# zenustech/zpc

Hardware: AMD Instinct MI355X
Metric: particle*steps/s (P2G+G2P) (higher is better)
Workload: dtype f32

## Files before the change

include/zs_rocm.h:

```cpp
#ifndef ZS_ROCM_H
#define ZS_ROCM_H
#include <stdbool.h>
#include <stddef.h>
#include <stdint.h>

#ifdef __cplusplus
extern "C" {
#endif

#if defined(__GNUC__)
#  define ZS_ROCM_EXPORT __attribute__((visibility("default")))
#else
#  define ZS_ROCM_EXPORT
#endif

typedef struct zs_rocm_policy zs_rocm_policy;

ZS_ROCM_EXPORT zs_rocm_policy *policy__device(void);
ZS_ROCM_EXPORT void del_policy__device(zs_rocm_policy *);
ZS_ROCM_EXPORT void zs_rocm_policy_sync(zs_rocm_policy *, int sync);
ZS_ROCM_EXPORT void zs_rocm_policy_profile(zs_rocm_policy *, int profile);
ZS_ROCM_EXPORT void zs_rocm_policy_device(zs_rocm_policy *, int procid);
ZS_ROCM_EXPORT void zs_rocm_policy_stream(zs_rocm_policy *, int streamid);
ZS_ROCM_EXPORT void zs_rocm_policy_listen(zs_rocm_policy *, int incomingProc, int incomingStreamid);
// ... 570 lines not shown
ZS_ROCM_EXPORT int zs_rocm_mesh_system_blocks(zs_rocm_policy *, const zs_rocm_mesh *, const zs_rocm_mesh_system *, float *scratch, float *elastic,
                                              float *barrier, float *friction, float *combined, float *inverse, int *status);
ZS_ROCM_EXPORT int zs_rocm_mesh_system_multiply(zs_rocm_policy *, const zs_rocm_mesh *, const zs_rocm_mesh_system *, float *scratch,
                                                const float *x, float *q);
ZS_ROCM_EXPORT int zs_rocm_mesh_system_solve(zs_rocm_policy *, const zs_rocm_mesh *, const zs_rocm_mesh_system *, float *scratch,
                                             const float *inverse, const float *b, float *x, int maxIters, float tol, float relTol,
                                             int checkEvery, void *record);
ZS_ROCM_EXPORT int zs_rocm_mesh_potential_sizes(const zs_rocm_mesh *, const zs_rocm_mesh_system *, size_t *sizes);
ZS_ROCM_EXPORT int zs_rocm_mesh_potential_evaluate(zs_rocm_policy *, const zs_rocm_mesh *, const zs_rocm_mesh_system *, const float *target,
                                                   const float *start, const float *verts, float *scratch, float *energies, double *parts,
                                                   float *grad, int *status);
ZS_ROCM_EXPORT int zs_rocm_mesh_potential_line_search(zs_rocm_policy *, const zs_rocm_mesh *, const zs_rocm_mesh_system *, const float *target,
                                                      const float *start, const float *verts, const float *dir, float tMax,
                                                      const float *tMaxDev, float c1, float shrink, int maxTrials, int checkEvery,
                                                      float *scratch, float *energies, float *x, void *record);
ZS_ROCM_EXPORT int zs_rocm_mesh_ccd(zs_rocm_policy *, const zs_rocm_mesh *, const float *verts, const float *dir, const int *ptPairs, size_t npt,
                                    const int *eePairs, size_t nee, float slack, float tMax, int maxIter, float *ptToi, float *eeToi,
                                    float *tMin, int *status);
#define ZS_ROCM_SLOT_STATUS_WORDS (8 + 2 * 256)
ZS_ROCM_EXPORT size_t zs_rocm_mpm_slot_outbox_bytes(size_t nbins, int outboxCap, int which);
ZS_ROCM_EXPORT void zs_rocm_mpm_build_neighbors27(zs_rocm_policy *, const zs_rocm_bht_3 *, int *nbr27 , int keyStride);
ZS_ROCM_EXPORT int zs_rocm_mpm_slot_particles(zs_rocm_policy *, const zs_rocm_bht_3 *, zs_rocm_attr pos, size_t n, float dx, int side,
                                              int keyIsOrigin, int K, const float *src, float *dst, int C, unsigned *cellMask, int *status);
ZS_ROCM_EXPORT size_t zs_rocm_mpm_slot_list(zs_rocm_policy *, const unsigned *cellMask, size_t nbins, int K, int *slots);
typedef struct zs_rocm_slot_storage {
  unsigned *cellMask;
  int K;
  const int *nbr;
  const int *nbr27;
  int *moverCount;
  unsigned *claim;
  float *moverRec;
  int outboxCap;
  int *status;
  const unsigned char *blockEdge;
} zs_rocm_slot_storage;
ZS_ROCM_EXPORT void zs_rocm_mpm_partition_edge(zs_rocm_policy *, const zs_rocm_bht_3 *, unsigned char *edge , int keyStride,
                                               int lo, int hi);
ZS_ROCM_EXPORT void zs_rocm_mpm_slot_compute_sparsity(zs_rocm_policy *, const zs_rocm_bht_3 *oldTab, const unsigned *cellMask, size_t nblocksOld,
                                                      int side, int keyIsOrigin, zs_rocm_bht_3 *newTab);
ZS_ROCM_EXPORT int zs_rocm_mpm_reslot(zs_rocm_policy *, const zs_rocm_bht_3 *oldTab, const zs_rocm_bht_3 *newTab, int side, int K, int C,
                                      const float *oldBuf, float *newBuf, const unsigned *oldMask, unsigned *newMask, const float *oldGrid,
                                      float *newGrid, int *status);
ZS_ROCM_EXPORT int zs_rocm_mpm_g2p2g_slots(zs_rocm_policy *, const zs_rocm_mpm_params *, zs_rocm_particles, const zs_rocm_bht_3 *,
                                           const float *gridA, float *gridB, size_t nblocks, const zs_rocm_slot_storage *st, int writeAll,
                                           size_t blockBegin, size_t blockEnd, int finish);
// ... 62 lines not shown
                                                                    const size_t *peerOffset, const size_t *peerCount, const int *blocks,
                                                                    size_t total);
typedef struct zs_rocm_mpm_step {
  const zs_rocm_mpm_params *params;
  zs_rocm_particles particles;
  const zs_rocm_bht_3 *table;
  const float *gridA;
  float *gridB;
  size_t nblocks;
  const zs_rocm_slot_storage *storage;
  int writeAll;
  float extf[3];
  float *maxVelSqr;
  const zs_rocm_collider *collider;
  size_t nBoundary;
  zs_rocm_dist *dist;
  zs_rocm_halo_plan *plan;
  zs_rocm_policy *commPolicy;
  float *haloGrid;
  void *evTransferBegin, *evTransferEnd;
  void **evBreakdown;
  int haloChannels;
  int rangeSchedule;
  float *handoverSnapshot;
  float *gridClear;
  int gridBIsClear;
  const zs_rocm_levelset *levelset;
} zs_rocm_mpm_step;
#define ZS_ROCM_STEP_EVENTS 8
#define ZS_ROCM_RANGES_IN_TURN 0
#define ZS_ROCM_RANGES_SIDE_BY_SIDE 1
#define ZS_ROCM_RANGES_ONE_LAUNCH 2
ZS_ROCM_EXPORT int zs_rocm_mpm_step_slotted(zs_rocm_policy *, const zs_rocm_mpm_step *);

#ifdef __cplusplus
}
#endif
#endif
```

zpc_amd/_lib.py:

```python
import ctypes as C
import os

_HERE = os.path.dirname(os.path.abspath(__file__))
LIB_PATH = os.path.join(_HERE, "lib", "libzsrocm.so")
if os.environ.get("ZS_ROCM_LIB"):
    LIB_PATH = os.environ["ZS_ROCM_LIB"]
    print("[zpc_amd] using HIP library %s" % LIB_PATH, flush=True)


class Port(C.Structure):
    _fields_ = [("base", C.c_void_p), ("idx", C.c_uint32), ("numTileBits", C.c_uint32),
                ("tileMask", C.c_uint32), ("numChns", C.c_uint32)]


class HashTableView(C.Structure):
    _fields_ = [("keys", C.c_void_p), ("indices", C.c_void_p), ("status", C.c_void_p), ("activeKeys", C.c_void_p),
                ("cnt", C.c_void_p), ("tableSize", C.c_int)]


class LBvhView(C.Structure):
    _fields_ = [("orderedBvs", C.c_void_p), ("parents", C.c_void_p), ("levels", C.c_void_p), ("leafInds", C.c_void_p),
                ("auxIndices", C.c_void_p), ("numNodes", C.c_int), ("numLeaves", C.c_int)]


# ... 14 lines not shown
class BhtViewLite(C.Structure):
    _fields_ = [("keys", C.c_void_p), ("indices", C.c_void_p), ("status", C.c_void_p), ("activeKeys", C.c_void_p),
                ("cnt", C.c_void_p), ("success", C.c_void_p), ("tableSize", C.c_uint32), ("numBuckets", C.c_uint32),
                ("hf0x", C.c_uint32), ("hf0y", C.c_uint32), ("hf1x", C.c_uint32), ("hf1y", C.c_uint32),
                ("hf2x", C.c_uint32), ("hf2y", C.c_uint32)]


class Particles(C.Structure):
    _fields_ = [("mass", Port), ("pos", Port), ("vel", Port), ("C", Port), ("F", Port), ("logJp", Port),
                ("stress", Port), ("n", C.c_size_t)]


class SlotStorage(C.Structure):
    _fields_ = [("cellMask", C.c_void_p), ("K", C.c_int), ("nbr", C.c_void_p), ("nbr27", C.c_void_p), ("moverCount", C.c_void_p),
                ("claim", C.c_void_p), ("moverRec", C.c_void_p), ("outboxCap", C.c_int), ("status", C.c_void_p),
                ("blockEdge", C.c_void_p)]


class MpmStep(C.Structure):
    _fields_ = [("params", C.c_void_p), ("particles", Particles), ("table", C.c_void_p), ("gridA", C.c_void_p), ("gridB", C.c_void_p),
                ("nblocks", C.c_size_t), ("storage", C.c_void_p), ("writeAll", C.c_int), ("extf", C.c_float * 3),
                ("maxVelSqr", C.c_void_p), ("collider", C.c_void_p), ("nBoundary", C.c_size_t), ("dist", C.c_void_p),
                ("plan", C.c_void_p), ("commPolicy", C.c_void_p), ("haloGrid", C.c_void_p), ("evTransferBegin", C.c_void_p),
                ("evTransferEnd", C.c_void_p), ("evBreakdown", C.POINTER(C.c_void_p)), ("haloChannels", C.c_int), ("rangeSchedule", C.c_int), ("handoverSnapshot", C.c_void_p),
                ("gridClear", C.c_void_p), ("gridBIsClear", C.c_int), ("levelset", C.c_void_p)]


class MpmParams(C.Structure):
    _fields_ = [("model", C.c_int), ("dx", C.c_float), ("dt", C.c_float), ("volume", C.c_float), ("E", C.c_float),
                ("nu", C.c_float), ("cohesion", C.c_float), ("beta", C.c_float), ("yieldSurface", C.c_float),
                ("volCorrection", C.c_int), ("side", C.c_int), ("keyIsOrigin", C.c_int), ("yieldStress", C.c_float),
                ("xi", C.c_float), ("Msqr", C.c_float), ("hardeningOn", C.c_int), ("bulk", C.c_float), ("viscosity", C.c_float)]


_lib = None


def lib():
    global _lib
    if _lib is None:
        if not os.path.exists(LIB_PATH):
            raise RuntimeError(
                "libzsrocm.so not built (%s): run `python -m zpc_amd.build` -- zpc_amd has no CPU fallback" % LIB_PATH)
        try:
            import torch
        except ImportError:
            pass
# ... 280 lines not shown
    PP = C.POINTER(MpmParams)
    L.zs_rocm_mpm_compute_sparsity.argtypes = [vp, vp, Port, sz, f32, i32, i32]
    L.zs_rocm_mpm_enlarge_sparsity.argtypes = [vp, vp, C.POINTER(C.c_int), C.POINTER(C.c_int), i32]
    L.zs_rocm_mpm_bin_particles.argtypes = [vp, vp, Port, sz, f32, i32, i32, vp, vp, vp]
    L.zs_rocm_mpm_build_neighbors.argtypes = [vp, vp, vp, i32]
    L.zs_rocm_mpm_p2g.argtypes = [vp, PP, Particles, vp, vp, sz, vp, vp, vp]
    L.zs_rocm_mpm_owner_rank.argtypes = [vp, Port, sz, f32, C.POINTER(C.c_int), C.POINTER(C.c_int), C.POINTER(C.c_int), i32, vp]
    L.zs_rocm_mpm_owner_counts.argtypes = [vp, vp, sz, i32, vp]
    L.zs_rocm_mpm_owner_counts.restype = None
    L.zs_rocm_mpm_g2p2g.argtypes = [vp, PP, Particles, vp, vp, vp, sz, vp, vp, vp, i32]
    L.zs_rocm_mpm_g2p2g_range.argtypes = [vp, PP, Particles, vp, vp, vp, sz, vp, vp, vp, i32, sz, sz, vp]
    L.zs_rocm_mpm_g2p2g_slotted.argtypes = [vp, PP, Particles, vp, vp, vp, sz, vp, i32, vp, vp, vp, vp, vp, i32, i32, vp]
    L.zs_rocm_mpm_g2p2g_slotted.restype = i32
    L.zs_rocm_mpm_g2p2g_slotted_range.argtypes = [vp, PP, Particles, vp, vp, vp, sz, vp, i32, vp, vp, vp, vp, vp, i32, i32, vp, sz, sz, i32]
    L.zs_rocm_mpm_g2p2g_slotted_range.restype = i32
    L.zs_rocm_mpm_g2p2g_slots.argtypes = [vp, PP, Particles, vp, vp, vp, sz, C.POINTER(SlotStorage), i32, sz, sz, i32]
    L.zs_rocm_mpm_g2p2g_slots.restype = i32
    L.zs_rocm_mpm_partition_edge.argtypes = [vp, vp, vp, i32, i32, i32]
    L.zs_rocm_mpm_slot_compute_sparsity.argtypes = [vp, vp, vp, sz, i32, i32, vp]
    L.zs_rocm_mpm_reslot.argtypes = [vp, vp, vp, i32, i32, i32, vp, vp, vp, vp, vp, vp, vp]
    L.zs_rocm_mpm_reslot.restype = i32
    L.zs_rocm_mpm_step_slotted.argtypes = [vp, C.POINTER(MpmStep)]
    L.zs_rocm_mpm_step_slotted.restype = i32
    L.zs_rocm_dist_halo_plan_from_lists.argtypes = [vp, i32, i32, C.POINTER(C.c_int), C.POINTER(C.c_size_t), C.POINTER(C.c_size_t),
                                                    C.POINTER(C.c_int), sz]
    L.zs_rocm_dist_halo_plan_from_lists.restype = vp
    L.zs_rocm_mpm_g2p2g_reorder_range.argtypes = [vp, PP, Particles, Particles, vp, vp, vp, vp, sz, vp, vp, vp, i32, sz, sz, vp]
    L.zs_rocm_mpm_grid_update.argtypes = [vp, PP, vp, sz, C.POINTER(C.c_float), vp]
    L.zs_rocm_mpm_g2p.argtypes = [vp, PP, Particles, vp, vp, sz, vp, vp, vp]
    L.zs_rocm_mpm_p2c2g.argtypes = [vp, PP, Particles, vp, vp, vp, sz, i32]
    L.zs_rocm_mpm_p2c2g.restype = i32
    L.zs_rocm_mpm_pre_g2c2p.argtypes = [vp, Particles]
    L.zs_rocm_mpm_g2c2p.argtypes = [vp, PP, Particles, vp, vp, vp, sz]
    L.zs_rocm_mpm_g2c2p.restype = i32
    L.zs_rocm_mpm_post_g2c2p.argtypes = [vp, PP, Particles]
    L.zs_rocm_mpm_g2c2p_step.argtypes = [vp, PP, Particles, vp, vp, sz]
    L.zs_rocm_mpm_g2c2p_step.restype = i32
    L.zs_rocm_mpm_stress.argtypes = [vp, PP, vp, vp, sz, vp]
    L.zs_rocm_mpm_update_stress.argtypes = [vp, PP, Particles]
    L.zs_rocm_svd3.argtypes = [vp, vp, sz, vp, vp, vp]
    L.zs_rocm_nacc_msqr.argtypes = [f32]
    L.zs_rocm_nacc_msqr.restype = f32
    L.zs_rocm_collider_init.argtypes = [C.POINTER(Collider), i32, i32, C.POINTER(C.c_float), i32]
    L.zs_rocm_mpm_apply_boundary.argtypes = [vp, PP, vp, vp, sz, C.POINTER(Collider)]
    L.zs_rocm_collider_resolve.argtypes = [vp, C.POINTER(Collider), vp, vp, sz, vp]
    L.zs_rocm_mpm_implicit_force.argtypes = [vp, PP, Particles, vp, sz, vp, vp, vp, vp, vp, vp]
# ... 111 lines not shown
```

zpc_amd/csrc/common.hpp:

```cpp
#pragma once
#include <hip/hip_runtime.h>

#include <cstdint>
#include <cstdio>
#include <cstdlib>
#include <map>
#include <mutex>
#include <vector>

#include "../../include/zs_rocm.h"

namespace zsr {

constexpr int kWave = 64;
constexpr int kNumSpareStreams = 32;
constexpr size_t kCtlBytes = 132 << 10;
constexpr size_t kCtlDesc8 = 32 << 10, kCtlTicket = 128 << 10;
constexpr size_t kCtlScanTiles = 4096;

struct DeviceContext {
  int dev = 0;
  hipStream_t streams[kNumSpareStreams] = {};
  hipEvent_t events[kNumSpareStreams + 1] = {};
  int errorStatus = 0;
// ... 71 lines not shown
  unsigned cu_count();
};

template <class T> struct Port {
  T *base;
  uint32_t idx, bits, mask, chns;
  __host__ __device__ __forceinline__ size_t off(size_t i) const {
    size_t j = (size_t)idx + i;
    return (((j >> bits) * (size_t)chns) << bits) | (j & (size_t)mask);
  }
  __host__ __device__ __forceinline__ T &operator[](size_t i) const { return base[off(i)]; }
  __host__ __device__ __forceinline__ size_t cstride() const { return (size_t)mask + 1; }
  __host__ __device__ bool contiguous() const { return chns == 1; }
};
template <class T, class P> inline Port<T> make_port(const P &p) {
  return Port<T>{(T *)p.base, p.idx, p.numTileBits, p.tileMask, p.numChns};
}
template <class T> inline Port<T> contiguous_port(T *p) { return Port<T>{p, 0u, 0u, 0u, 1u}; }

inline unsigned ceil_div(size_t a, size_t b) { return (unsigned)((a + b - 1) / b); }

int mpm_g2p2g_slots_signal(zs_rocm_policy *pol, const zs_rocm_mpm_params *p, zs_rocm_particles ps, const zs_rocm_bht_3 *tab, const float *gridA,
                           float *gridB, size_t nblocks, const zs_rocm_slot_storage *st, int writeAll, size_t blockBegin, size_t blockEnd, int finish,
                           unsigned long long *signal, size_t signalBlocks, float *gridClear, float *zeroWord);
bool levelset_collider_ok(const zs_rocm_collider *collider, const zs_rocm_levelset *levelset);
void levelset_blocks_enqueue(hipStream_t stream, const zs_rocm_mpm_params *p, const int *activeKeys, float *grid, size_t nblocks,
                             const zs_rocm_collider *collider, const zs_rocm_levelset *levelset, float *dof);
bool levelset_ok(const zs_rocm_levelset *levelset);
bool transition_collider_ok(const zs_rocm_collider *collider, const zs_rocm_levelset_transition *transition);
bool transition_blocks_enqueue(hipStream_t stream, const zs_rocm_mpm_params *p, const int *activeKeys, float *grid, size_t nblocks,
                               const zs_rocm_collider *collider, const zs_rocm_levelset_transition *transition, float *dof);

}

namespace zsr {

__device__ __forceinline__ int lane_id() { return (int)(threadIdx.x & 63); }
__device__ __forceinline__ int wave_id() { return (int)(threadIdx.x >> 6); }

template <class T> __device__ __forceinline__ T shfl_down(T v, int d) { return __shfl_down(v, d, 64); }
template <class T> __device__ __forceinline__ T shfl_up(T v, int d) { return __shfl_up(v, d, 64); }
template <class T> __device__ __forceinline__ T shfl(T v, int l) { return __shfl(v, l, 64); }

__device__ __forceinline__ unsigned long long lanemask_lt() {
  return (1ull << (threadIdx.x & 63)) - 1ull;
}

// ... 10 lines not shown
```

zpc_amd/csrc/dist.hip:

```cpp
#include <rccl/rccl.h>

#include <algorithm>
#include <cstring>
#include <utility>
#include <vector>

#include "common.hpp"

struct zs_rocm_dist {
  ncclComm_t comm = nullptr;
  int rank = 0, world = 1, device = 0;
  bool broken = false;
};

namespace zsr {
static int nccl_check(ncclResult_t r, const char *what, const char *file, int line) {
  if (r == ncclSuccess) return 0;
  fprintf(stderr, "[zs_rocm | rccl] %s failed: %s at %s:%d\n", what, ncclGetErrorString(r), file, line);
  report_error(hipErrorUnknown, what, file, line);
  return -1;
}
#define ZSR_NCCL(expr)                                               \
  do {                                                               \
    if (::zsr::nccl_check((expr), #expr, __FILE__, __LINE__)) return -1; \
// ... 324 lines not shown
  return 0;
}

}
static __global__ void step_gate_kernel(const unsigned long long *signal, unsigned long long target) {
  const unsigned long long t0 = wall_clock64();
  while (__hip_atomic_load(signal, __ATOMIC_RELAXED, __HIP_MEMORY_SCOPE_AGENT) < target) {
    __builtin_amdgcn_s_sleep(64);
    if (wall_clock64() - t0 > 1000000000ull) __builtin_trap();
  }
}
extern "C" {

int zs_rocm_mpm_step_slotted(zs_rocm_policy *pol, const zs_rocm_mpm_step *a) {
  if (!pol || !a || !a->params || !a->table || !a->gridA || !a->gridB || !a->storage) return -1;
  if (a->levelset && !zsr::levelset_collider_ok(a->collider, a->levelset)) return -1;
  const size_t nb = a->nblocks;
  if (!nb) return 0;
  const int side = a->params->side;
  const size_t gridBytes = nb * (size_t)7 * side * side * side * sizeof(float);
  if (a->haloChannels < 0 || a->haloChannels > 7) return -1;
  if (a->rangeSchedule < ZS_ROCM_RANGES_IN_TURN || a->rangeSchedule > ZS_ROCM_RANGES_ONE_LAUNCH) return -1;
  if (a->rangeSchedule == ZS_ROCM_RANGES_ONE_LAUNCH && side != 8) return -1;
  float *const gridClear = side == 8 ? a->gridClear : nullptr;
  if (gridClear && (gridClear == a->gridA || gridClear == a->gridB || ((uintptr_t)gridClear & 15u))) return -1;
  if (!(gridClear && a->gridBIsClear)) zs_rocm_memset(pol, a->gridB, 0, gridBytes);
  float *const hgrid = a->haloGrid ? a->haloGrid : a->gridB;
  const bool exchange = a->dist && a->plan && a->plan->total;
  auto slots = [&](zs_rocm_policy *on, size_t b0, size_t b1, int finish, unsigned long long *signal, size_t signalBlocks) {
    return mpm_g2p2g_slots_signal(on, a->params, a->particles, a->table, a->gridA, a->gridB, nb, a->storage, a->writeAll, b0, b1, finish, signal,
                                  signalBlocks, gridClear, finish ? a->maxVelSqr : nullptr);
  };
  const int hch = a->haloChannels ? a->haloChannels : 7;
  const bool overlap = exchange && a->commPolicy && a->nBoundary > 0 && a->nBoundary < nb;
  int rc = 0;
  auto stamp = [&](void *ev) {
    if (!ev) return;
    Launch L(pol, "step: event");
    ZSR_CHECK(hipEventRecord((hipEvent_t)ev, L.stream));
  };
  auto bd = [&](int k, zs_rocm_policy *on) {
    if (!a->evBreakdown || !a->evBreakdown[k]) return;
    Launch L(on, "step: breakdown event");
    ZSR_CHECK(hipEventRecord((hipEvent_t)a->evBreakdown[k], L.stream));
  };
  stamp(a->evTransferBegin);
  bd(0, pol);
  if (overlap) {
    zs_rocm_halo_plan *p = a->plan;
    if (!p->evBoundary || !p->evDone) {
      DeviceGuard guard(p->device);
      if (!p->evBoundary && hipEventCreateWithFlags(&p->evBoundary, hipEventDisableTiming) != hipSuccess) p->evBoundary = nullptr;
      if (!p->evDone && hipEventCreateWithFlags(&p->evDone, hipEventDisableTiming) != hipSuccess) p->evDone = nullptr;
      if (!p->evBoundary || !p->evDone) {
// ... 110 lines not shown
```

zpc_amd/csrc/mpm_slot.hpp:

```cpp
#pragma once
#include "mpm_arena.hpp"
#include "mpm_fused_common.hpp"

namespace zsr {

constexpr int SL_REC = 48;
constexpr int SLR_DCELL = 14, SLR_FLAG = 15, SLR_V = 16, SLR_C = 19, SLR_PF = 28;

struct SlotArgs {
  const float *gridA;
  float *gridB;
  unsigned *cellMask;
  int K;
  const int *nbr;
  const int *nbr27;
  int *moverCount;
  unsigned *claim;
  float *moverRec;
  int *status;
  int binBase, nbins, nbinsAll;
  int cap;
  const unsigned char *blockEdge;
  unsigned long long *signal;
  int signalBlocks;
  float *gridClear;
};

constexpr int SL_NCTR = 256, SL_SENT = 8, SL_DELIVERED = 8 + SL_NCTR;
__device__ __forceinline__ int neighbour_bin8(const int *row27, int blk, int sub, int code) {
  if (code == 13) return blk * 8 + sub;
  const int dd[3] = {code / 9 - 1, (code / 3) % 3 - 1, code % 3 - 1};
  int sx[3] = {((sub >> 2) & 1) + dd[0], ((sub >> 1) & 1) + dd[1], (sub & 1) + dd[2]}, bo[3];
#pragma unroll
  for (int d = 0; d < 3; ++d) {
    bo[d] = sx[d] < 0 ? -1 : (sx[d] > 1 ? 1 : 0);
    sx[d] &= 1;
  }
  const int nb = row27[(bo[0] + 1) * 9 + (bo[1] + 1) * 3 + (bo[2] + 1)];
  return nb < 0 ? -1 : nb * 8 + ((sx[0] * 2 + sx[1]) * 2 + sx[2]);
}

constexpr int SL_NG = 9;
constexpr int SL_KMAX = 32;
constexpr int SL_ARRQ = 4;
constexpr int SL_XQ = 64;

__device__ __forceinline__ int nth_low_bit(unsigned w, unsigned t) {
  for (unsigned k = 0; k < t && w; ++k) w &= w - 1u;
  return w ? __ffs((int)w) - 1 : -1;
}
struct SlotShared {
  float *varena;
  float *parena;
  float *stage;
  unsigned long long *smask;
  unsigned short *tab;
  unsigned *mask0;
  unsigned *clr;
  unsigned *arrLocal;
  const int *nbrBlk;
  const int *nbrBin;
  unsigned (*arrCnt)[64];
  unsigned short (*arrQ)[64][SL_ARRQ];
  unsigned *xCnt;
  unsigned (*xq)[SL_XQ];
  int *outCount, *sent, *homed, *xOver;
};

template <int SIDE, class FM, class FV, class FC, class FP>
__device__ __forceinline__ void scatter_node_task(const MpmDev &mp, int node, int ch, const int (&nc)[3], const float (&d0)[3], FM fm, FV fv, FC fC,
                                                  FP fP, const int *nbrBlk, float *gridB, int *status) {
  constexpr int NC = SIDE * SIDE * SIDE;
// ... 451 lines not shown
```

zpc_amd/csrc/mpm_slotblk.hip:

```cpp
#include "mpm_slot.hpp"
#ifdef ZS_SLOTBLK_CHECK_ARENA
#include <cassert>
#endif

namespace zsr {

constexpr int SB_NG = 5;
constexpr int SB_MAXCH = 64;
constexpr int LIST_CS = 3;

struct SubGeom {
  int o[3], org[3];
};
__device__ __forceinline__ SubGeom sub_geom(const int (&borg)[3], int b) {
  SubGeom g;
  g.o[0] = ((b >> 2) & 1) * 4;
  g.o[1] = ((b >> 1) & 1) * 4;
  g.o[2] = (b & 1) * 4;
#pragma unroll
  for (int d = 0; d < 3; ++d) g.org[d] = borg[d] + g.o[d];
  return g;
}

struct BlkShared {
// ... 356 lines not shown
  constexpr int NC = 512;
  __shared__ float s_varena[3 * ArenaBlk::CH];
  __shared__ float s_parena[7 * ArenaBin8::CH];
  __shared__ float s_stage[SB_NG * G2P2G_QF * 64];
  __shared__ unsigned long long s_smask[SB_NG];
  __shared__ unsigned short s_tab[2][SL_KMAX * 64];
  __shared__ unsigned s_masks[8][64];
  __shared__ unsigned s_clr[2][64], s_arrLocal[8][64], s_arrCnt[3][64];
  __shared__ unsigned short s_arrQ[3][64][SL_ARRQ];
  __shared__ unsigned s_xCnt[3], s_xq[3][SL_XQ];
  __shared__ int s_nbrBlk[27], s_nbrBin[2][27], s_nbr8[8];
  __shared__ int s_cnt[2][4];
  __shared__ int s_total[8], s_gbase[8], s_binQ[8], s_oc[8];
  __shared__ unsigned char s_chBin[SB_MAXCH], s_chIdx[SB_MAXCH];
  __shared__ unsigned s_desc[SB_MAXCH + 5];
  __shared__ unsigned s_done, s_listDone, s_faces[2];
  __shared__ int s_sums[3], s_G;
  __shared__ float *s_clear;
  const BlkShared sh{s_varena, s_parena, s_stage, s_smask, s_tab, s_masks, s_clr, s_arrLocal, s_arrCnt, s_arrQ, s_xCnt, s_xq, s_nbrBlk, s_nbrBin, s_nbr8,
                     s_cnt, s_oc, s_desc, &s_done, &s_listDone, s_faces, s_sums};
  const int tid = threadIdx.x, lane = tid & 63, w = tid >> 6;
  const int blk = (int)blockIdx.x + A.binBase / 8;
  const int bin0 = blk * 8;
  const unsigned mask = A.cellMask[(size_t)(bin0 + w) * 64 + lane];
  s_masks[w][lane] = mask;
  s_arrLocal[w][lane] = 0u;
  {
    int n = __popc(mask);
#pragma unroll
    for (int sft = 32; sft >= 1; sft >>= 1) n += __shfl_xor(n, sft, 64);
    if (lane == 0) s_total[w] = n;
  }
  if (tid < 128) s_clr[tid >> 6][tid & 63] = 0u;
  if (tid < 192) s_arrCnt[tid >> 6][tid & 63] = 0u;
  if (tid < 3) {
    s_xCnt[tid] = 0u;
    s_sums[tid] = 0;
  }
  if (tid < 8) (&s_cnt[0][0])[tid] = 0;
  if (tid == 0) {
    s_done = 0u;
    s_listDone = 0u;
    s_clear = A.gridClear ? A.gridClear + (size_t)blk * 7 * NC : nullptr;
  }
  if (tid >= 64 && tid < 64 + 27) s_nbrBlk[tid - 64] = A.nbr27[(size_t)blk * 27 + (tid - 64)];
  if (tid >= 96 && tid < 104) s_nbr8[tid - 96] = A.nbr[(size_t)blk * 8 + (tid - 96)];
  int borg[3];
// ... 113 lines not shown
```

zpc_amd/csrc/mpm_slotted.hip:

```cpp
#include "mpm_slot.hpp"

namespace zsr {

void exclusive_scan_u32(Launch &L, const unsigned *in, size_t n, unsigned *out);

template <int SIDE>
static __global__ __launch_bounds__(256) void slot_assign_kernel(BhtDev t, Port<float> pos, size_t n, float dx, unsigned *cellCount, int K,
                                                                 int *srcOf, int *status, int kscale) {
  size_t i = (size_t)blockIdx.x * blockDim.x + threadIdx.x;
  if (i >= n) return;
  float p[3];
  load_attr<3>(pos, i, p);
  int key[3], loc[3];
#pragma unroll
  for (int d = 0; d < 3; ++d) {
    const int c = (int)floorf(p[d] * (1.0f / dx) - 0.5f);
    loc[d] = c & (SIDE - 1);
    key[d] = (c - loc[d]) / SIDE * kscale;
  }
  const int b = bht_query<3>(t, key);
  if (b < 0) {
    status[2] = 1;
    return;
  }
// ... 201 lines not shown
        C[d] = rc[SLR_C + d];
        PF[d] = rc[SLR_PF + d];
      }
      pstore<LW, 3>(ps.vel, o, v);
      pstore<LW, 9>(ps.C, o, C);
      {
        float S[STRESS_N];
        stress_pack(PF, S);
        pstore<LW, STRESS_N>(ps.stress, o, S);
      }
    }
  }
#pragma unroll
  for (int sft = 32; sft >= 1; sft >>= 1) nhomed += __shfl_xor(nhomed, sft, 64);
  if ((threadIdx.x & 63) == 0 && nhomed) atomicAdd(&status[SL_DELIVERED + (int)((bin >> 3) & (SL_NCTR - 1))], nhomed);
}

static __global__ __launch_bounds__(256) void slot_commit_kernel(unsigned *cellMask, unsigned *claim, size_t ncells, int K, float *zeroWord) {
  const size_t c = (size_t)blockIdx.x * blockDim.x + threadIdx.x;
  if (c == 0 && zeroWord) *zeroWord = 0.f;
  if (c >= ncells) return;
  const unsigned tk = claim[c], clr = claim[ncells + c];
  if (!tk && !clr) return;
  const unsigned m0 = cellMask[c];
  const unsigned kmask = K >= 32 ? 0xffffffffu : ((1u << K) - 1u);
  const unsigned n = (tk >> 16) + (tk & 0xffffu);
  unsigned rest = ~m0 & kmask, bits = 0u;
  for (unsigned k = 0; k < n && rest; ++k) {
    const unsigned b = rest & (0u - rest);
    bits |= b;
    rest ^= b;
  }
  cellMask[c] = (m0 & ~clr) | bits;
  claim[c] = 0u;
  claim[ncells + c] = 0u;
}

template <int SIDE>
static __global__ __launch_bounds__(256) void slot_sparsity_kernel(BhtDev oldT, const unsigned *cellMask, size_t ncells, int kscale, BhtDev newT) {
  const size_t c = (size_t)blockIdx.x * blockDim.x + threadIdx.x;
  const bool valid = c < ncells && cellMask[c] != 0u;
  int b[3] = {0, 0, 0};
  if (valid) {
    const size_t bin = c >> 6;
    const int lane = (int)(c & 63), blk = (int)(bin / bins_per_block<SIDE>()), sub = (int)(bin % bins_per_block<SIDE>());
    const int o[3] = {SIDE == 4 ? 0 : ((sub >> 2) & 1) * 4, SIDE == 4 ? 0 : ((sub >> 1) & 1) * 4, SIDE == 4 ? 0 : (sub & 1) * 4};
    const int l[3] = {lane >> 4, (lane >> 2) & 3, lane & 3};
#pragma unroll
    for (int d = 0; d < 3; ++d) b[d] = floordiv(oldT.activeKeys[3 * (size_t)blk + d] * (SIDE / kscale) + o[d] + l[d] - 1, SIDE) * kscale;
  }
  const int px = shfl_up(b[0], 1), py = shfl_up(b[1], 1), pz = shfl_up(b[2], 1);
  const bool pvalid = shfl_up((int)valid, 1) != 0;
  const bool dup = lane_id() != 0 && pvalid && px == b[0] && py == b[1] && pz == b[2];
  if (valid && !dup) bht_insert<3>(newT, b);
}
static __global__ __launch_bounds__(256) void reslot_map_kernel(BhtDev oldT, int nOld, BhtDev newT, int *map) {
// ... 74 lines not shown
  hipLaunchKernelGGL(slot_mask_kernel, dim3(ceil_div(ncells, 256)), dim3(256), 0, L.stream, cellMask, ncells, K);
  hipLaunchKernelGGL(slot_gather_kernel, dim3(ceil_div(nslots, 256)), dim3(256), 0, L.stream, src, dst, nslots, C, (const int *)srcOf);
  return 0;
}

size_t zs_rocm_mpm_slot_list(zs_rocm_policy *pol, const unsigned *cellMask, size_t nbins, int K, int *slots) {
  Launch L(pol, "slot_list");
  const size_t ncells = nbins * 64;
  if (!ncells) return 0;
  unsigned *cnt = (unsigned *)L.temp(sizeof(unsigned) * (ncells + 1)), *start = (unsigned *)L.temp(sizeof(unsigned) * (ncells + 1));
  ZSR_CHECK(hipMemsetAsync(cnt + ncells, 0, sizeof(unsigned), L.stream));
  hipLaunchKernelGGL(slot_popc_kernel, dim3(ceil_div(ncells, 256)), dim3(256), 0, L.stream, cellMask, ncells, cnt);
  exclusive_scan_u32(L, cnt, ncells + 1, start);
  unsigned total = 0;
  ZSR_CHECK(hipMemcpyAsync(&total, start + ncells, sizeof(unsigned), hipMemcpyDeviceToHost, L.stream));
  if (slots) hipLaunchKernelGGL(slot_emit_kernel, dim3(ceil_div(ncells, 256)), dim3(256), 0, L.stream, cellMask, (const unsigned *)start, ncells, K, slots);
  ZSR_CHECK(hipStreamSynchronize(L.stream));
  return (size_t)total;
}

int zs_rocm_mpm_g2p2g_slots(zs_rocm_policy *pol, const zs_rocm_mpm_params *p, zs_rocm_particles ps, const zs_rocm_bht_3 *tab,
                            const float *gridA, float *gridB, size_t nblocks, const zs_rocm_slot_storage *st, int writeAll,
                            size_t blockBegin, size_t blockEnd, int finish) {
  return zsr::mpm_g2p2g_slots_signal(pol, p, ps, tab, gridA, gridB, nblocks, st, writeAll, blockBegin, blockEnd, finish, nullptr, 0, nullptr, nullptr);
}
}
namespace zsr {
int mpm_g2p2g_slots_signal(zs_rocm_policy *pol, const zs_rocm_mpm_params *p, zs_rocm_particles ps, const zs_rocm_bht_3 *tab, const float *gridA,
                           float *gridB, size_t nblocks, const zs_rocm_slot_storage *st, int writeAll, size_t blockBegin, size_t blockEnd, int finish,
                           unsigned long long *signal, size_t signalBlocks, float *gridClear, float *zeroWord) {
  if (!st) return -1;
  if (signal && p->side != 8) return -1;
  if (p->side != 8) gridClear = nullptr;
  if (gridClear && (gridClear == gridA || gridClear == gridB || ((uintptr_t)gridClear & 15u))) return -1;
  unsigned *const cellMask = st->cellMask;
  const int K = st->K, outboxCap = st->outboxCap;
  const int *const nbr = st->nbr, *const nbr27 = st->nbr27;
  int *const moverCount = st->moverCount, *const status = st->status;
  unsigned *const claim = st->claim;
  float *const moverRec = st->moverRec;
  if (!nblocks) return 0;
  if (!cellMask || !nbr || !nbr27 || !moverCount || !claim || !moverRec || !status || K < 1 || K > 32 || outboxCap < 1 || outboxCap > (1 << 20)) return -1;
  if (p->model < ZS_MPM_FIXED_COROTATED || p->model > ZS_MPM_EQUATION_OF_STATE) return -1;
  if (uniform_lane_width(ps, model_uses_logjp(p->model), writeAll != 0) != 64 || (writeAll && (!ps.vel.base || !ps.C.base))) {
    fprintf(stderr, "[zs_rocm] g2p2g_slotted needs all particle attributes in one TileVector<f32, 64>\n");
    return -1;
  }
  if (blockEnd > nblocks) blockEnd = nblocks;
  Launch L(pol, "G2P2GTransfer(slotted)");
  MpmDev mp = make_dev(p);
  ParticlesDev pd = make_particles(ps);
  BhtDev t = tab->t.dev();
  const unsigned bpb = p->side == 4 ? 1u : 8u;
  const unsigned nbinsAll = (unsigned)(nblocks * bpb);
  const unsigned nbins = blockBegin < blockEnd ? (unsigned)((blockEnd - blockBegin) * bpb) : 0u;
  const SlotArgs A{gridA, gridB, cellMask, K, nbr, nbr27, moverCount, claim, moverRec, status, (int)(blockBegin * bpb), (int)nbins, (int)nbinsAll, outboxCap,
                   st->blockEdge, signal, (int)signalBlocks, gridClear};
#define CALL_REHOME3(M, WA)                                                                                                              \
  hipLaunchKernelGGL((slot_rehome_kernel<model_is_fluid(M), model_uses_logjp(M), WA>), dim3(ceil_div((size_t)nbinsAll, 32)), dim3(256), 0,  \
                     L.stream, pd, (const unsigned *)cellMask, claim, (const int *)moverCount, (const float *)moverRec, outboxCap,        \
                     (size_t)nbinsAll, K, status)
#define CALL_REHOME(SS, M)                      \
  do {                                          \
    if (writeAll) { CALL_REHOME3(M, true); }    \
    else { CALL_REHOME3(M, false); }            \
  } while (0)
  if (p->side == 8) {
    if (nbins) launch_g2p2g_slotblk(L.stream, p->model, writeAll != 0, mp, pd, t, A);
  } else if (nbins) {
#define CALL_SLOT4(SS, M)                                                                                                  \
  do {                                                                                                                     \
    if (writeAll) hipLaunchKernelGGL((g2p2g_slot_kernel<4, M, true>), dim3(nbins), dim3(512), 0, L.stream, mp, pd, t, A);  \
    else hipLaunchKernelGGL((g2p2g_slot_kernel<4, M, false>), dim3(nbins), dim3(512), 0, L.stream, mp, pd, t, A);          \
  } while (0)
    ZSR_DISPATCH_PURE_(4, p->model, CALL_SLOT4)
  }
  if (finish) ZSR_DISPATCH_PURE_(0, p->model, CALL_REHOME)
  if (finish) {
    const size_t ncells = (size_t)nbinsAll * 64;
    hipLaunchKernelGGL(slot_commit_kernel, dim3(ceil_div(ncells, 256)), dim3(256), 0, L.stream, cellMask, claim, ncells, K, zeroWord);
  }
  return 0;
}
}
extern "C" {

int zs_rocm_mpm_g2p2g_slotted_range(zs_rocm_policy *pol, const zs_rocm_mpm_params *p, zs_rocm_particles ps, const zs_rocm_bht_3 *tab,
                                    const float *gridA, float *gridB, size_t nblocks, unsigned *cellMask, int K, const int *nbr, const int *nbr27,
                                    int *moverCount, unsigned *claim, float *moverRec, int outboxCap, int writeAll, int *status,
                                    size_t blockBegin, size_t blockEnd, int finish) {
  const zs_rocm_slot_storage st{cellMask, K, nbr, nbr27, moverCount, claim, moverRec, outboxCap, status, nullptr};
  return zs_rocm_mpm_g2p2g_slots(pol, p, ps, tab, gridA, gridB, nblocks, &st, writeAll, blockBegin, blockEnd, finish);
}

int zs_rocm_mpm_g2p2g_slotted(zs_rocm_policy *pol, const zs_rocm_mpm_params *p, zs_rocm_particles ps, const zs_rocm_bht_3 *tab, const float *gridA,
                              float *gridB, size_t nblocks, unsigned *cellMask, int K, const int *nbr, const int *nbr27, int *moverCount,
                              unsigned *claim, float *moverRec, int outboxCap, int writeAll, int *status) {
  return zs_rocm_mpm_g2p2g_slotted_range(pol, p, ps, tab, gridA, gridB, nblocks, cellMask, K, nbr, nbr27, moverCount, claim, moverRec, outboxCap,
                                         writeAll, status, 0, nblocks, 1);
}

void zs_rocm_mpm_partition_edge(zs_rocm_policy *pol, const zs_rocm_bht_3 *tab, unsigned char *edge, int keyStride, int lo, int hi) {
  Launch L(pol, "partition_edge");
// ... 39 lines not shown
```

zpc_amd/mpm.py:

```python
import ctypes as C

import torch

from ._lib import lib, Port, Particles, MpmParams, SlotStorage, MpmStep
from .containers import Bht

FIXED_COROTATED, DRUCKER_PRAGER, VONMISES_FIXED_COROTATED, NACC = 0, 1, 2, 3
EQUATION_OF_STATE = 4
HAS_LOGJP = (DRUCKER_PRAGER, NACC)


class MpmTransfer:
    def __init__(self, pol, n, dx, dt, model=FIXED_COROTATED, side=4, lane_width=64, E=5e4, nu=0.4, volume=1.0,
                 cohesion=0.0, beta=1.0, yield_surface=0.816496580927726 * 2.0 * 0.5 / (3.0 - 0.5), vol_correction=True,
                 device="cuda", key_is_origin=False, aos=False, cache_stress=False, yield_stress=240e6, xi=0.8, friction_angle=45.0,
                 hardening=True, bulk=4e4, viscosity=0.0):
        self.pol, self.n, self.L, self.side = pol, int(n), int(lane_width), int(side)
        self.device = torch.device(device)
        self.model = model
        self.fluid = model == EQUATION_OF_STATE
        self.nF = 1 if self.fluid else 9
        self.nchn = 16 + self.nF + (1 if model in HAS_LOGJP else 0)
        self.off = {"m": 0, "x": 1, "v": 4, "C": 7, "F": 16, "logJp": 25}
        self.cache_stress = bool(cache_stress)
# ... 9 lines not shown
        self.buf = torch.zeros(self.tiles * self.L * self.nchn, dtype=torch.float32, device=self.device)
        self.buf2 = None
        self.drift_flag = None
        self.drift_tripped = False
        self.outside_tripped = False
        self.key_is_origin = bool(key_is_origin)
        self.kstride = side if key_is_origin else 1
        self.params = MpmParams(model, dx, dt, volume, E, nu, cohesion, beta, yield_surface, int(vol_correction), side,
                                int(self.key_is_origin), yield_stress, xi, lib().zs_rocm_nacc_msqr(friction_angle), int(hardening),
                                bulk, viscosity)
        self.table = None
        self.grid = None
        self.grid2 = self.grid3 = None
        self._clean_grid = None
        self.rotate_grids = True
        self.nblocks = 0
        self.order = self.bin_start = self.cell_count = self.nbr = None
        self.binned = False
        self.slotted = False
        self.n_slots = 0
        self.K = 0
        self.slot_record = {"sent": 0, "homed": 0, "flags": [0] * 5, "periods": 0, "edge_periods": 0, "log": []}

    def _grids_written(self):
        self._clean_grid = None

    def _zero(self, t):
        lib().zs_rocm_memset(self.pol.handle, t.data_ptr(), 0, t.numel() * t.element_size())

    def _port(self, name, buf=None):
        buf = self.buf if buf is None else buf
        bits = self.L.bit_length() - 1
        return Port(buf.data_ptr() + self.off[name] * self.L * 4, 0, bits, self.L - 1, self.nchn)

    def particles(self, buf=None):
        null = Port(None, 0, 0, 0, 1)
        return Particles(self._port("m", buf), self._port("x", buf), self._port("v", buf), self._port("C", buf), self._port("F", buf),
                         self._port("logJp", buf) if self.model in HAS_LOGJP else null,
                         self._port("PF", buf) if self.cache_stress else null, self.n_slots if self.slotted else self.n)

    def set_particles(self, buf, n):
        self.n = int(n)
        self.tiles = (self.n + self.L - 1) // self.L
        assert buf.numel() == self.tiles * self.L * self.nchn
        self.buf, self.buf2 = buf, None
        self.order = self.bin_start = self.cell_count = None
# ... 463 lines not shown
        L.zs_rocm_mpm_post_g2c2p(self.pol.handle, C.byref(self.params), self.particles())
        self.binned = False

    def g2p2g(self, write_all=False, split=None, between=None, reorder=False):
        self._grids_written()
        if self.slotted:
            if reorder:
                raise ValueError("slotted storage: no re-ordering steps (the step keeps the order itself)")
            if getattr(self, "grid2", None) is None or self.grid2.numel() != self.grid.numel():
                self.grid2 = torch.zeros_like(self.grid)
            else:
                self._zero(self.grid2)
            src, dst = self.grid, self.grid2
            self.grid, self.grid2 = dst, src
            ranges = [(0, self.nblocks)] if not split else [(0, int(split)), (int(split), self.nblocks)]
            for k, (b0, b1) in enumerate(ranges):
                rc = lib().zs_rocm_mpm_g2p2g_slots(self.pol.handle, C.byref(self.params), self.particles(), self.table.handle, src.data_ptr(),
                                                   dst.data_ptr(), self.nblocks, C.byref(self.slot_storage), int(write_all),
                                                   b0, b1, int(k == len(ranges) - 1))
                if rc != 0:
                    raise RuntimeError("zs_rocm_mpm_g2p2g_slotted refused the call")
                if k == 0 and between is not None:
                    between()
            return
        if not (self.cache_stress and self.binned):
            raise RuntimeError("g2p2g needs cache_stress=True and rebin()")
        src_buf = None
        if reorder and write_all:
            raise ValueError("a re-ordering step cannot also materialise v, C, stress (write_all)")
        if reorder:
            L = lib()
            if self.order is None or self.order.numel() != self.n:
                self.order = torch.empty(self.n, dtype=torch.int32, device=self.device)
            L.zs_rocm_mpm_bin_particles(self.pol.handle, self.table.handle, self._port("x"), self.n, self.params.dx, self.side,
                                        int(self.key_is_origin), self.order.data_ptr(), self.bin_start.data_ptr(),
                                        self.cell_count.data_ptr())
            if self.buf2 is None:
                self.buf2 = torch.empty_like(self.buf)
            src_buf, self.buf, self.buf2 = self.buf, self.buf2, self.buf
        if getattr(self, "grid2", None) is None or self.grid2.numel() != self.grid.numel():
            self.grid2 = torch.zeros_like(self.grid)
        else:
            self._zero(self.grid2)
        if self.drift_flag is None:
            self.drift_flag = torch.zeros(3, dtype=torch.int32, device=self.device)
        ranges = [(0, self.nblocks)] if not split else [(0, int(split)), (int(split), self.nblocks)]
# ... 42 lines not shown
            a = self._step_args = MpmStep()
        a.params = C.addressof(self.params)
        a.particles = self.particles()
        a.table = self.table.handle
        a.gridA, a.gridB = src.data_ptr(), dst.data_ptr()
        a.gridClear = clr.data_ptr() if clr is not None else None
        a.gridBIsClear = int(dst_is_clear)
        a.nblocks = self.nblocks
        a.storage = C.addressof(self.slot_storage)
        a.writeAll = int(write_all)
        a.extf = (C.c_float * 3)(*extf)
        a.maxVelSqr = max_vel.data_ptr() if max_vel is not None else None
        a.collider = C.addressof(collider) if collider is not None else None
        self._step_levelset = _levelset_view(levelset) if levelset is not None else None
        a.levelset = C.addressof(self._step_levelset) if levelset is not None else None
        a.nBoundary = int(n_boundary)
        a.dist = comm._h if comm is not None else None
        a.plan = plan._h if plan is not None else None
        a.commPolicy = comm_pol.handle if comm_pol is not None else None
        a.haloGrid = halo_grid.data_ptr() if halo_grid is not None else None
        a.haloChannels = int(halo_channels)
        a.rangeSchedule = int(range_schedule)
        a.handoverSnapshot = handover_snapshot.data_ptr() if handover_snapshot is not None else None
        a.evTransferBegin, a.evTransferEnd = (events[0], events[1]) if events is not None else (None, None)
        a.evBreakdown = breakdown if breakdown is not None else None
        if getattr(self, "_poisoned", False):
            raise RuntimeError("this MpmTransfer is poisoned: an earlier zs_rocm_mpm_step_slotted failed after committing the particle side of its step")
        if lib().zs_rocm_mpm_step_slotted(self.pol.handle, C.byref(a)) != 0:
            self._poisoned = True
            raise RuntimeError("zs_rocm_mpm_step_slotted failed: the step is half applied (particles advanced, grids not): this object cannot be stepped again")
        if rotate:
            self.grid, self.grid2, self.grid3 = dst, clr, src
            self._clean_grid = (clr, self.table)
        else:
            self.grid, self.grid2 = dst, src

    def margin_violated(self):
        return self.drift_tripped or (self.drift_flag is not None and bool(self.drift_flag[0].item()))

    def left_partition(self):
        return self.outside_tripped or (self.drift_flag is not None and bool(self.drift_flag[2].item()))

    def exact_path_particles(self, reset=True):
        if self.drift_flag is None:
            return 0
        c = int(self.drift_flag[1].item())
        if reset:
            self._zero(self.drift_flag[1:2])
        return c

    def reorder_partition(self, first_mask):
        import numpy as np
        keys = self.active_keys()
# ... 138 lines not shown
```

Baseline: 11.26 billion.

## Defer slot commit into next step's slot kernel prologue

```diff
diff --git a/include/zs_rocm.h b/include/zs_rocm.h
--- a/include/zs_rocm.h
+++ b/include/zs_rocm.h
@@ -616,6 +616,7 @@
 ZS_ROCM_EXPORT void zs_rocm_mpm_build_neighbors27(zs_rocm_policy *, const zs_rocm_bht_3 *, int *nbr27 , int keyStride);
 ZS_ROCM_EXPORT int zs_rocm_mpm_slot_particles(zs_rocm_policy *, const zs_rocm_bht_3 *, zs_rocm_attr pos, size_t n, float dx, int side,
                                               int keyIsOrigin, int K, const float *src, float *dst, int C, unsigned *cellMask, int *status);
+ZS_ROCM_EXPORT int zs_rocm_mpm_slot_commit(zs_rocm_policy *, unsigned *cellMask, unsigned *claim, size_t nbins, int K);
 ZS_ROCM_EXPORT size_t zs_rocm_mpm_slot_list(zs_rocm_policy *, const unsigned *cellMask, size_t nbins, int K, int *slots);
 typedef struct zs_rocm_slot_storage {
   unsigned *cellMask;
@@ -724,6 +725,7 @@
   void **evBreakdown;
   int haloChannels;
   int rangeSchedule;
+  int deferCommit;
   float *handoverSnapshot;
   float *gridClear;
   int gridBIsClear;
diff --git a/zpc_amd/_lib.py b/zpc_amd/_lib.py
--- a/zpc_amd/_lib.py
+++ b/zpc_amd/_lib.py
@@ -60,7 +60,7 @@
                 ("nblocks", C.c_size_t), ("storage", C.c_void_p), ("writeAll", C.c_int), ("extf", C.c_float * 3),
                 ("maxVelSqr", C.c_void_p), ("collider", C.c_void_p), ("nBoundary", C.c_size_t), ("dist", C.c_void_p),
                 ("plan", C.c_void_p), ("commPolicy", C.c_void_p), ("haloGrid", C.c_void_p), ("evTransferBegin", C.c_void_p),
-                ("evTransferEnd", C.c_void_p), ("evBreakdown", C.POINTER(C.c_void_p)), ("haloChannels", C.c_int), ("rangeSchedule", C.c_int), ("handoverSnapshot", C.c_void_p),
+                ("evTransferEnd", C.c_void_p), ("evBreakdown", C.POINTER(C.c_void_p)), ("haloChannels", C.c_int), ("rangeSchedule", C.c_int), ("deferCommit", C.c_int), ("handoverSnapshot", C.c_void_p),
                 ("gridClear", C.c_void_p), ("gridBIsClear", C.c_int), ("levelset", C.c_void_p)]
 
 
@@ -387,6 +387,8 @@
     L.zs_rocm_mpm_reslot.restype = i32
     L.zs_rocm_mpm_step_slotted.argtypes = [vp, C.POINTER(MpmStep)]
     L.zs_rocm_mpm_step_slotted.restype = i32
+    L.zs_rocm_mpm_slot_commit.argtypes = [vp, vp, vp, sz, i32]
+    L.zs_rocm_mpm_slot_commit.restype = i32
     L.zs_rocm_dist_halo_plan_from_lists.argtypes = [vp, i32, i32, C.POINTER(C.c_int), C.POINTER(C.c_size_t), C.POINTER(C.c_size_t),
                                                     C.POINTER(C.c_int), sz]
     L.zs_rocm_dist_halo_plan_from_lists.restype = vp
diff --git a/zpc_amd/csrc/common.hpp b/zpc_amd/csrc/common.hpp
--- a/zpc_amd/csrc/common.hpp
+++ b/zpc_amd/csrc/common.hpp
@@ -117,7 +117,7 @@
 
 int mpm_g2p2g_slots_signal(zs_rocm_policy *pol, const zs_rocm_mpm_params *p, zs_rocm_particles ps, const zs_rocm_bht_3 *tab, const float *gridA,
                            float *gridB, size_t nblocks, const zs_rocm_slot_storage *st, int writeAll, size_t blockBegin, size_t blockEnd, int finish,
-                           unsigned long long *signal, size_t signalBlocks, float *gridClear, float *zeroWord);
+                           unsigned long long *signal, size_t signalBlocks, float *gridClear, float *zeroWord, int deferCommit);
 bool levelset_collider_ok(const zs_rocm_collider *collider, const zs_rocm_levelset *levelset);
 void levelset_blocks_enqueue(hipStream_t stream, const zs_rocm_mpm_params *p, const int *activeKeys, float *grid, size_t nblocks,
                              const zs_rocm_collider *collider, const zs_rocm_levelset *levelset, float *dof);
diff --git a/zpc_amd/csrc/dist.hip b/zpc_amd/csrc/dist.hip
--- a/zpc_amd/csrc/dist.hip
+++ b/zpc_amd/csrc/dist.hip
@@ -370,6 +370,7 @@
   if (a->haloChannels < 0 || a->haloChannels > 7) return -1;
   if (a->rangeSchedule < ZS_ROCM_RANGES_IN_TURN || a->rangeSchedule > ZS_ROCM_RANGES_ONE_LAUNCH) return -1;
   if (a->rangeSchedule == ZS_ROCM_RANGES_ONE_LAUNCH && side != 8) return -1;
+  if (a->deferCommit && side != 8) return -1;
   float *const gridClear = side == 8 ? a->gridClear : nullptr;
   if (gridClear && (gridClear == a->gridA || gridClear == a->gridB || ((uintptr_t)gridClear & 15u))) return -1;
   if (!(gridClear && a->gridBIsClear)) zs_rocm_memset(pol, a->gridB, 0, gridBytes);
@@ -377,7 +378,7 @@
   const bool exchange = a->dist && a->plan && a->plan->total;
   auto slots = [&](zs_rocm_policy *on, size_t b0, size_t b1, int finish, unsigned long long *signal, size_t signalBlocks) {
     return mpm_g2p2g_slots_signal(on, a->params, a->particles, a->table, a->gridA, a->gridB, nb, a->storage, a->writeAll, b0, b1, finish, signal,
-                                  signalBlocks, gridClear, finish ? a->maxVelSqr : nullptr);
+                                  signalBlocks, gridClear, a->maxVelSqr, a->deferCommit != 0);
   };
   const int hch = a->haloChannels ? a->haloChannels : 7;
   const bool overlap = exchange && a->commPolicy && a->nBoundary > 0 && a->nBoundary < nb;
diff --git a/zpc_amd/csrc/mpm_slot.hpp b/zpc_amd/csrc/mpm_slot.hpp
--- a/zpc_amd/csrc/mpm_slot.hpp
+++ b/zpc_amd/csrc/mpm_slot.hpp
@@ -24,6 +24,7 @@
   unsigned long long *signal;
   int signalBlocks;
   float *gridClear;
+  float *zeroWord;
 };
 
 constexpr int SL_NCTR = 256, SL_SENT = 8, SL_DELIVERED = 8 + SL_NCTR;
@@ -48,6 +49,16 @@
 __device__ __forceinline__ int nth_low_bit(unsigned w, unsigned t) {
   for (unsigned k = 0; k < t && w; ++k) w &= w - 1u;
   return w ? __ffs((int)w) - 1 : -1;
+}
+__host__ __device__ __forceinline__ unsigned slot_commit_word(unsigned m0, unsigned tickets, unsigned cleared, unsigned kmask) {
+  const unsigned n = (tickets >> 16) + (tickets & 0xffffu);
+  unsigned rest = ~m0 & kmask, bits = 0u;
+  for (unsigned k = 0; k < n && rest; ++k) {
+    const unsigned b = rest & (0u - rest);
+    bits |= b;
+    rest ^= b;
+  }
+  return (m0 & ~cleared) | bits;
 }
 struct SlotShared {
   float *varena;
diff --git a/zpc_amd/csrc/mpm_slotblk.hip b/zpc_amd/csrc/mpm_slotblk.hip
--- a/zpc_amd/csrc/mpm_slotblk.hip
+++ b/zpc_amd/csrc/mpm_slotblk.hip
@@ -402,7 +402,19 @@
   const int tid = threadIdx.x, lane = tid & 63, w = tid >> 6;
   const int blk = (int)blockIdx.x + A.binBase / 8;
   const int bin0 = blk * 8;
-  const unsigned mask = A.cellMask[(size_t)(bin0 + w) * 64 + lane];
+  unsigned mask;
+  {
+    const size_t c = (size_t)(bin0 + w) * 64 + lane, ncells = (size_t)A.nbinsAll * 64;
+    mask = A.cellMask[c];
+    const unsigned tk = A.claim[c], clr = A.claim[ncells + c];
+    if (tk | clr) {
+      mask = slot_commit_word(mask, tk, clr, A.K >= 32 ? 0xffffffffu : ((1u << A.K) - 1u));
+      A.cellMask[c] = mask;
+      A.claim[c] = 0u;
+      A.claim[ncells + c] = 0u;
+    }
+  }
+  if (blk == 0 && tid == 0 && A.zeroWord) *A.zeroWord = 0.f;
   s_masks[w][lane] = mask;
   s_arrLocal[w][lane] = 0u;
   {
diff --git a/zpc_amd/csrc/mpm_slotted.hip b/zpc_amd/csrc/mpm_slotted.hip
--- a/zpc_amd/csrc/mpm_slotted.hip
+++ b/zpc_amd/csrc/mpm_slotted.hip
@@ -247,16 +247,8 @@
   if (c >= ncells) return;
   const unsigned tk = claim[c], clr = claim[ncells + c];
   if (!tk && !clr) return;
-  const unsigned m0 = cellMask[c];
   const unsigned kmask = K >= 32 ? 0xffffffffu : ((1u << K) - 1u);
-  const unsigned n = (tk >> 16) + (tk & 0xffffu);
-  unsigned rest = ~m0 & kmask, bits = 0u;
-  for (unsigned k = 0; k < n && rest; ++k) {
-    const unsigned b = rest & (0u - rest);
-    bits |= b;
-    rest ^= b;
-  }
-  cellMask[c] = (m0 & ~clr) | bits;
+  cellMask[c] = slot_commit_word(cellMask[c], tk, clr, kmask);
   claim[c] = 0u;
   claim[ncells + c] = 0u;
 }
@@ -377,15 +369,24 @@
 int zs_rocm_mpm_g2p2g_slots(zs_rocm_policy *pol, const zs_rocm_mpm_params *p, zs_rocm_particles ps, const zs_rocm_bht_3 *tab,
                             const float *gridA, float *gridB, size_t nblocks, const zs_rocm_slot_storage *st, int writeAll,
                             size_t blockBegin, size_t blockEnd, int finish) {
-  return zsr::mpm_g2p2g_slots_signal(pol, p, ps, tab, gridA, gridB, nblocks, st, writeAll, blockBegin, blockEnd, finish, nullptr, 0, nullptr, nullptr);
+  return zsr::mpm_g2p2g_slots_signal(pol, p, ps, tab, gridA, gridB, nblocks, st, writeAll, blockBegin, blockEnd, finish, nullptr, 0, nullptr, nullptr, 0);
+}
+
+int zs_rocm_mpm_slot_commit(zs_rocm_policy *pol, unsigned *cellMask, unsigned *claim, size_t nbins, int K) {
+  if (!pol || !cellMask || !claim || K < 1 || K > 32) return -1;
+  if (!nbins) return 0;
+  Launch L(pol, "slot_commit");
+  const size_t ncells = nbins * 64;
+  hipLaunchKernelGGL(slot_commit_kernel, dim3(ceil_div(ncells, 256)), dim3(256), 0, L.stream, cellMask, claim, ncells, K, (float *)nullptr);
+  return 0;
 }
 }
 namespace zsr {
 int mpm_g2p2g_slots_signal(zs_rocm_policy *pol, const zs_rocm_mpm_params *p, zs_rocm_particles ps, const zs_rocm_bht_3 *tab, const float *gridA,
                            float *gridB, size_t nblocks, const zs_rocm_slot_storage *st, int writeAll, size_t blockBegin, size_t blockEnd, int finish,
-                           unsigned long long *signal, size_t signalBlocks, float *gridClear, float *zeroWord) {
+                           unsigned long long *signal, size_t signalBlocks, float *gridClear, float *zeroWord, int deferCommit) {
   if (!st) return -1;
-  if (signal && p->side != 8) return -1;
+  if ((signal || deferCommit) && p->side != 8) return -1;
   if (p->side != 8) gridClear = nullptr;
   if (gridClear && (gridClear == gridA || gridClear == gridB || ((uintptr_t)gridClear & 15u))) return -1;
   unsigned *const cellMask = st->cellMask;
@@ -410,7 +411,7 @@
   const unsigned nbinsAll = (unsigned)(nblocks * bpb);
   const unsigned nbins = blockBegin < blockEnd ? (unsigned)((blockEnd - blockBegin) * bpb) : 0u;
   const SlotArgs A{gridA, gridB, cellMask, K, nbr, nbr27, moverCount, claim, moverRec, status, (int)(blockBegin * bpb), (int)nbins, (int)nbinsAll, outboxCap,
-                   st->blockEdge, signal, (int)signalBlocks, gridClear};
+                   st->blockEdge, signal, (int)signalBlocks, gridClear, p->side == 8 ? zeroWord : nullptr};
 #define CALL_REHOME3(M, WA)                                                                                                              \
   hipLaunchKernelGGL((slot_rehome_kernel<model_is_fluid(M), model_uses_logjp(M), WA>), dim3(ceil_div((size_t)nbinsAll, 32)), dim3(256), 0,  \
                      L.stream, pd, (const unsigned *)cellMask, claim, (const int *)moverCount, (const float *)moverRec, outboxCap,        \
@@ -431,9 +432,10 @@
     ZSR_DISPATCH_PURE_(4, p->model, CALL_SLOT4)
   }
   if (finish) ZSR_DISPATCH_PURE_(0, p->model, CALL_REHOME)
-  if (finish) {
+  if (finish && !deferCommit) {
     const size_t ncells = (size_t)nbinsAll * 64;
-    hipLaunchKernelGGL(slot_commit_kernel, dim3(ceil_div(ncells, 256)), dim3(256), 0, L.stream, cellMask, claim, ncells, K, zeroWord);
+    hipLaunchKernelGGL(slot_commit_kernel, dim3(ceil_div(ncells, 256)), dim3(256), 0, L.stream, cellMask, claim, ncells, K,
+                       p->side == 8 ? nullptr : zeroWord);
   }
   return 0;
 }
diff --git a/zpc_amd/mpm.py b/zpc_amd/mpm.py
--- a/zpc_amd/mpm.py
+++ b/zpc_amd/mpm.py
@@ -55,6 +55,27 @@
         self.K = 0
         self.slot_record = {"sent": 0, "homed": 0, "flags": [0] * 5, "periods": 0, "edge_periods": 0, "log": []}
 
+    defer_commit = True
+    _commit_pending = False
+    _cell_mask = None
+
+    @property
+    def cell_mask(self):
+        if self._commit_pending:
+            self.flush_commit()
+        return self._cell_mask
+
+    @cell_mask.setter
+    def cell_mask(self, t):
+        self._cell_mask = t
+        self._commit_pending = False
+
+    def flush_commit(self):
+        self._commit_pending = False
+        if lib().zs_rocm_mpm_slot_commit(self.pol.handle, self._cell_mask.data_ptr(), self.mover_dest.data_ptr(), self.nbins, self.K) != 0:
+            raise RuntimeError("zs_rocm_mpm_slot_commit refused its arguments")
+        self.pol.syncCtx()
+
     def _grids_written(self):
         self._clean_grid = None
 
@@ -564,6 +585,7 @@
                     raise RuntimeError("zs_rocm_mpm_g2p2g_slotted refused the call")
                 if k == 0 and between is not None:
                     between()
+            self._commit_pending = False
             return
         if not (self.cache_stress and self.binned):
             raise RuntimeError("g2p2g needs cache_stress=True and rebin()")
@@ -652,6 +674,7 @@
         a.haloChannels = int(halo_channels)
         a.rangeSchedule = int(range_schedule)
         a.handoverSnapshot = handover_snapshot.data_ptr() if handover_snapshot is not None else None
+        a.deferCommit = int(self.side == 8 and self.defer_commit)
         a.evTransferBegin, a.evTransferEnd = (events[0], events[1]) if events is not None else (None, None)
         a.evBreakdown = breakdown if breakdown is not None else None
         if getattr(self, "_poisoned", False):
@@ -659,6 +682,7 @@
         if lib().zs_rocm_mpm_step_slotted(self.pol.handle, C.byref(a)) != 0:
             self._poisoned = True
             raise RuntimeError("zs_rocm_mpm_step_slotted failed: the step is half applied (particles advanced, grids not): this object cannot be stepped again")
+        self._commit_pending = bool(a.deferCommit)
         if rotate:
             self.grid, self.grid2, self.grid3 = dst, clr, src
             self._clean_grid = (clr, self.table)
```

Result: no change. 11.35 billion, median of 6 (+0.8%).
